# Sukikui/PTI-LDM-VAE

Hardware: AMD Instinct MI355X
Metric: vae_train_images_per_sec_256x256 (higher is better)
Workload: dtype fp16 forward operands + activations / bf16 backward operands + gradients, fp32 accumulate; 1 GPU; config/vae_dente_no_adv.json 256x256x1 batch 32/GPU: fwd + L1 + 1e-3*KL + bwd + all-reduce + Adam (perceptual term omitted: --perceptual times it; adversarial branch inactive before epoch 6, --adv times it); global_batch=32, parallelism=dp1

## Files before the change

pti_ldm_vae_amd/csrc/conv_common.h:

```cpp
#pragma once
#include "pti_common.h"

namespace pti_conv {

struct ConvArgs {
  const bf16* x;
  const unsigned char* w;
  const float* bias;
  const stat_t* in_stats;
  const float* gamma;
  const float* beta;
  const bf16* res;
  bf16* y;
  stat_t* out_stats;
  int N, H, W, Cin, Ho, Wo, Cout;
  int mode, prologue, groups, out_groups;
  float eps, inv_cnt;
  int tiles_x, tiles_y;
  int gn_mode;
  int g_groups;
  float g_inv_cnt, g_eps;
  const stat_t* g_stats; const float* g_gamma; const float* g_beta;
  float* g_sums;
  int g_T;
  bf16* act_out;
  int in_f16, res_f16, out_f16;
  int pool2;
  int relu_out;
  int w_f16;
  const bf16* x2;
  const float* p_sums;
  int x2_f16;
};
constexpr int PRO_GNB = 3;

typedef _Float16 f16x8 __attribute__((ext_vector_type(8)));
template <bool OPH>
__device__ __forceinline__ f32x16 mfma32(const bf16x8& a, const bf16x8& b, const f32x16& c) {
  if constexpr (OPH)
    return __builtin_amdgcn_mfma_f32_32x32x16_f16(__builtin_bit_cast(f16x8, a), __builtin_bit_cast(f16x8, b), c, 0, 0, 0);
  else
    return __builtin_amdgcn_mfma_f32_32x32x16_bf16(a, b, c, 0, 0, 0);
}

__host__ __device__ constexpr int pick_ck2(int cin, int ct) {
  const int ck = cin % 128 == 0 ? 128 : (cin % 64 == 0 ? 64 : 32);
  const int cap = ct >= 128 ? 128 : (ct == 64 ? 64 : 32);
  return ck < cap ? ck : cap;
}

template <int NV, int N, int O>
__device__ __forceinline__ void fold32_level(float (&v)[NV], int j) {
  if constexpr (O >= 1) {
    if constexpr (N > 1) {
      const bool hi = (j & O) != 0;
// ... 50 lines not shown
```

pti_ldm_vae_amd/csrc/conv_mfma.hip:

```cpp
#include "conv_common.h"

namespace {
using namespace pti_conv;

constexpr int TH = 8, TW = 16;

__host__ __device__ constexpr int pick_cout_tile(int cout) { return cout % 128 == 0 ? 128 : (cout % 64 == 0 ? 64 : 32); }
__host__ __device__ constexpr int pick_ck(int cin, int stride2) {
  int ck = cin % 128 == 0 ? 128 : (cin % 64 == 0 ? 64 : 32);
  return (stride2 && ck > 64) ? 64 : ck;
}
__host__ __device__ constexpr int pick_wblk(int kbc, int nt) {
  int best = 1;
  for (int w = 1; w <= kbc; ++w)
    if (kbc % w == 0 && w * nt <= 16) best = w;
  return best;
}

template <int KS, int S, int CK, int COUT_TILE>
struct Cfg {
  static constexpr int HH = (TH - 1) * S + KS, HW = (TW - 1) * S + KS;
  static constexpr int NP = HH * HW;
  static constexpr int NC = CK / 8;
  static constexpr int PIXB = CK * 2;
// ... 242 lines not shown
              b1 += __shfl_xor(b1, o, 64);
              b2 += __shfl_xor(b2, o, 64);
            }
            if (j == 0) {
              const int g = co / 2;
              stat_add(&sstat[2 * g], a1);
              stat_add(&sstat[2 * g + 1], a2);
              stat_add(&sstat[2 * g + 2], b1);
              stat_add(&sstat[2 * g + 3], b2);
            }
          }
        }
      }
    }
  }
  if (do_stats) {
    __syncthreads();
    const int g0 = (ct * COUT_TILE) / ocpg, ng = COUT_TILE / ocpg;
    if (tid < 2 * ng)
      atomicAdd((unsigned long long*)&a.out_stats[(n * a.out_groups + g0) * 2 + tid], (unsigned long long)sstat[2 * g0 + tid]);
  }
}

template <int KS, int CK, int CT, int PXF, bool SAVE, int FM, int PRO>
__global__ __launch_bounds__(256, (PXF == 2 ? 4 : 2)) void conv_mfma2_kernel(ConvArgs a) {
  using C = Cfg2<KS, CK, CT, PXF>;
  const int prologue = PRO >= 0 ? PRO : a.prologue;
  const bool gn_on = FM == 3 ? true : (FM == 0 ? a.gn_mode != 0 : false);
  const bool in_f16 = FM == 0 ? (bool)a.in_f16 : (FM == 1);
  const bool res_f16 = FM == 0 ? (bool)a.res_f16 : (FM == 1 || FM == 3);
  const bool out_f16 = FM == 0 ? (bool)a.out_f16 : (FM == 1);
  constexpr bool OPH = (FM == 1);
  if (out_f16) fp16_saturate_on();
  __shared__ __attribute__((aligned(16))) unsigned char smem[C::LDS_BYTES];
  unsigned char* halo = smem;
  const int tid = threadIdx.x, lane = tid & 63, wave = tid >> 6;
  const int hsel = lane >> 5;
  int t = blockIdx.x;
  const int tile_x = t % a.tiles_x;
  t /= a.tiles_x;
  const int tile_y = t % a.tiles_y;
  const int n = t / a.tiles_y;
  const int oy0 = tile_y * C::TH2, ox0 = tile_x * C::TW2;
  const int ct = blockIdx.y;
  const int nchunks = a.Cin / CK;
  const int wm = wave / C::WN, wn = wave % C::WN;

  const int pad_lo = (a.mode == PTI_CONV_ZINS) ? 2 : (KS - 1) / 2;
  const int vy0 = oy0 - pad_lo, vx0 = ox0 - pad_lo;
  const bool twox = (a.mode == PTI_CONV_UP2) || (a.mode == PTI_CONV_ZINS);
  const int VH = twox ? 2 * a.H : a.H, VW = twox ? 2 * a.W : a.W;

  int pbase[KS], tkey[KS];
  {
    const int j = lane & 31, tx = j & 15, row0 = 2 * PXF * wm + (j >> 4);
#pragma unroll
    for (int kw = 0; kw < KS; ++kw) {
      const int hx = tx + kw;
      tkey[kw] = (hsel ^ ((hx >> C::KEY_SHIFT) & (C::NC - 1))) << 4;
      pbase[kw] = (row0 * C::HW + hx) * C::PIXB;
    }
// ... 397 lines not shown
  }
  if (gn_on) {
    if (tid < 2 * CT) {
      const float* gsm = reinterpret_cast<const float*>(smem + C::STAT_OFF);
      float v = gsm[tid];
#pragma unroll
      for (int m = 1; m < C::WM; ++m) v += gsm[m * 2 * CT + tid];
      a.g_sums[(((size_t)n * a.g_T + tile_y * a.tiles_x + tile_x) * a.Cout + ct * CT) * 2 + tid] = v;
    }
  } else if (do_stats) {
    const stat_t* sstat = reinterpret_cast<const stat_t*>(smem + C::STAT_OFF);
    const int g0 = (ct * CT) / ocpg, ng = CT / ocpg;
    if (tid < 2 * ng)
      atomicAdd((unsigned long long*)&a.out_stats[(n * a.out_groups + g0) * 2 + tid], (unsigned long long)sstat[2 * g0 + tid]);
  }
}

template <int KS, int CK, int CT, int PXF>
int launch2_cfg(ConvArgs a, hipStream_t st) {
  using C = Cfg2<KS, CK, CT, PXF>;
  a.tiles_x = cdiv(a.Wo, C::TW2);
  a.tiles_y = cdiv(a.Ho, C::TH2);
  a.g_T = a.tiles_x * a.tiles_y;
  dim3 grid(a.N * a.tiles_x * a.tiles_y, a.Cout / CT);
  const bool res = a.res != nullptr;
  const int fm = (a.w_f16 && a.in_f16 && a.out_f16 && (a.res_f16 || !res)) ? 1
               : (!a.in_f16 && !a.out_f16 && (!a.res_f16 || !res)) ? 2
               : (!a.in_f16 && !a.out_f16 && a.res_f16) ? 3 : 0;
  const bool fwd_silu = fm == 1 && a.prologue == PTI_PRO_GN_SILU && !a.gn_mode && !a.pool2;
  const bool fwd_plain = fm == 1 && a.prologue == PTI_PRO_NONE && !a.gn_mode && !a.pool2;
  const bool dgrad = fm == 2 && a.prologue == PTI_PRO_NONE && !a.gn_mode && !a.out_stats;
  const bool dgrad_gn = fm == 3 && a.prologue == PTI_PRO_NONE && a.gn_mode && !a.out_stats && !a.pool2;
  if (a.x2) {
    if constexpr (KS == 3 && PXF == 4 && CT == 128) {
      if (!(fm == 3 && a.gn_mode && a.act_out && !a.out_stats && !a.pool2 && a.mode == PTI_CONV_S1 && !a.relu_out)) return 4;
      PTI_LAUNCH((conv_mfma2_kernel<KS, CK, CT, PXF, true, 3, PRO_GNB>), grid, dim3(256), 0, st, a);
      return 0;
    } else {
      return 4;
    }
  }
  if (a.relu_out && !(fwd_plain && !a.act_out)) return 3;
  constexpr int FPRO = PXF == 4 ? PTI_PRO_GN_SILU : -1;
  const bool fwd_gn_rt = fm == 1 && a.prologue == PTI_PRO_GN && !a.gn_mode && !a.pool2 && FPRO < 0;
  if constexpr (KS == 3) {
    if (a.act_out) {
      if (fwd_silu || fwd_gn_rt) PTI_LAUNCH((conv_mfma2_kernel<KS, CK, CT, PXF, true, 1, FPRO>), grid, dim3(256), 0, st, a);
      else if (a.w_f16) return 2;
      else PTI_LAUNCH((conv_mfma2_kernel<KS, CK, CT, PXF, true, 0, -1>), grid, dim3(256), 0, st, a);
      return 0;
    }
  } else if (a.act_out) {
    return 1;
  }
  if (fwd_silu) PTI_LAUNCH((conv_mfma2_kernel<KS, CK, CT, PXF, false, 1, FPRO>), grid, dim3(256), 0, st, a);
  else if (fwd_plain) PTI_LAUNCH((conv_mfma2_kernel<KS, CK, CT, PXF, false, 1, PTI_PRO_NONE>), grid, dim3(256), 0, st, a);
  else if (fm == 1 && !a.gn_mode && !a.pool2) PTI_LAUNCH((conv_mfma2_kernel<KS, CK, CT, PXF, false, 1, -1>), grid, dim3(256), 0, st, a);
  else if (a.w_f16) return 2;
  else if (dgrad) PTI_LAUNCH((conv_mfma2_kernel<KS, CK, CT, PXF, false, 2, PTI_PRO_NONE>), grid, dim3(256), 0, st, a);
  else if (dgrad_gn) PTI_LAUNCH((conv_mfma2_kernel<KS, CK, CT, PXF, false, 3, PTI_PRO_NONE>), grid, dim3(256), 0, st, a);
  else PTI_LAUNCH((conv_mfma2_kernel<KS, CK, CT, PXF, false, 0, -1>), grid, dim3(256), 0, st, a);
  return 0;
}
template <int KS>
int launch2(const ConvArgs& a, int ck, int ct, hipStream_t st) {
  if (ct == 128) {
    if (ck == 128) return launch2_cfg<KS, 128, 128, 4>(a, st);
    if (ck == 64) return launch2_cfg<KS, 64, 128, 4>(a, st);
    return launch2_cfg<KS, 32, 128, 4>(a, st);
  }
  if (ct == 64) {
    if (ck == 64) return launch2_cfg<KS, 64, 64, 2>(a, st);
    return launch2_cfg<KS, 32, 64, 2>(a, st);
  }
  return launch2_cfg<KS, 32, 32, 2>(a, st);
}

struct PackArgs {
  const float* src[4];
  int nsrc;
  bf16* dst;
  int cout_l, cin_l;
  int cout_o, cin_o;
  int ks, ck, cout_tile, flip;
  int f16;
  long long total;
// ... 302 lines not shown
```

pti_ldm_vae_amd/csrc/groupnorm.hip:

```cpp
#include "pti_common.h"

namespace {

__global__ __launch_bounds__(256) void gn_stats_kernel(const bf16* __restrict__ x, stat_t* __restrict__ stats,
                                                       int HW, int C, int G, int pix_per_block, int x_f16) {
  extern __shared__ stat_t sm_q[];
  stat_t* sm = sm_q;
  const int n = blockIdx.y;
  const int tid = threadIdx.x;
  const int NC = C / 8;
  const int ppi = 256 / NC;
  const int lc = tid % NC, lp = tid / NC;
  for (int i = tid; i < 2 * G; i += 256) sm[i] = 0;
  __syncthreads();
  const int p0 = blockIdx.x * pix_per_block;
  const int p1 = min(p0 + pix_per_block, HW);
  float s[8], q[8];
#pragma unroll
  for (int j = 0; j < 8; ++j) s[j] = q[j] = 0.f;
  const bf16* base = x + (size_t)n * HW * C + lc * 8;
  int p = p0 + lp;
  for (; p + 3 * ppi < p1; p += 4 * ppi) {
    u32x4 r[4];
#pragma unroll
// ... 62 lines not shown
  int bps = cdiv(2048, n);
  int ppb = cdiv(hw, bps);
  if (ppb < 16 * ppi) ppb = 16 * ppi;
  ppb = cdiv(ppb, 4 * ppi) * 4 * ppi;
  bps = cdiv(hw, ppb);
  PTI_LAUNCH(gn_stats_kernel, dim3(bps, n), dim3(256), 2 * groups * sizeof(stat_t), (hipStream_t)s,
                     (const bf16*)x, (stat_t*)stats, hw, c, groups, ppb, x_f16);
  PTI_CHECK_LAUNCH("gn_stats");
  return PTI_OK;
}

namespace {

struct GnbArgs {
  const bf16* x; const bf16* da; const bf16* dres; bf16* dx;
  const stat_t* stats; const float* gamma; const float* beta;
  float* sums;
  float* dgamma; float* dbeta;
  int HW, C, G, silu, ppb;
  float eps, inv_cnt;
  int x_f16;
  int N;
  float* part;
};

__global__ __launch_bounds__(256) void gn_bwd_reduce_kernel(GnbArgs a) {
  extern __shared__ float sm[];
  const int n = blockIdx.y, tid = threadIdx.x;
  const int NC = a.C / 8, ppi = 256 / NC, lc = tid % NC, lp = tid / NC;
  for (int i = tid; i < 8 * a.C; i += 256) sm[i] = 0.f;
  __syncthreads();
  const int cpg = a.C / a.G;
  float sc[8], sh[8], mu[8], rs[8];
#pragma unroll
  for (int j = 0; j < 8; ++j) {
    const int ch = lc * 8 + j, g = ch / cpg;
    const float sum = stat_f(a.stats, (n * a.G + g) * 2), sq = stat_f(a.stats, (n * a.G + g) * 2 + 1);
    const float mean = sum * a.inv_cnt;
    const float rstd = rsqrtf(fmaxf(sq * a.inv_cnt - mean * mean, 0.f) + a.eps);
    mu[j] = mean; rs[j] = rstd;
    sc[j] = rstd * a.gamma[ch];
    sh[j] = a.beta[ch] - mean * sc[j];
  }
  float s1[8], s2[8];
#pragma unroll
  for (int j = 0; j < 8; ++j) s1[j] = s2[j] = 0.f;
// ... 68 lines not shown
    const float* p = part + (size_t)n * T * R + i;
    int t = w;
    for (; t + 48 < T; t += 64) {
      const float a0 = p[(size_t)t * R], a1 = p[(size_t)(t + 16) * R], a2 = p[(size_t)(t + 32) * R], a3 = p[(size_t)(t + 48) * R];
      v += (a0 + a1) + (a2 + a3);
    }
    for (; t < T; t += 16) v += p[(size_t)t * R];
  }
  red[w][lane] = v;
  __syncthreads();
  if (w == 0 && i < R) {
    float r[16];
#pragma unroll
    for (int k = 0; k < 16; ++k) r[k] = red[k][lane];
#pragma unroll
    for (int o = 8; o > 0; o >>= 1)
#pragma unroll
      for (int k = 0; k < o; ++k) r[k] += r[k + o];
    sums[(size_t)n * R + i] = r[0];
  }
}

__global__ __launch_bounds__(256) void gn_bwd_apply_kernel(GnbArgs a) {
  const int n = blockIdx.y, tid = threadIdx.x;
  const int NC = a.C / 8, ppi = 256 / NC, lc = tid % NC, lp = tid / NC;
  const int cpg = a.C / a.G;
  const int p0 = blockIdx.x * a.ppb, p1 = min(p0 + a.ppb, a.HW);
  const size_t base = (size_t)n * a.HW * a.C + lc * 8;
  constexpr int U = 4;
  u32x4 rx[U], rd[U], rr[U];
  auto load_batch = [&](int pb) {
#pragma unroll
    for (int u = 0; u < U; ++u) {
      const int p = pb + u * ppi;
      rx[u] = rd[u] = rr[u] = u32x4{0u, 0u, 0u, 0u};
      if (p < p1) {
        rx[u] = __builtin_nontemporal_load((const u32x4*)(a.x + base + (size_t)p * a.C));
        rd[u] = __builtin_nontemporal_load((const u32x4*)(a.da + base + (size_t)p * a.C));
        if (a.dres) rr[u] = __builtin_nontemporal_load((const u32x4*)(a.dres + base + (size_t)p * a.C));
      }
    }
  };
  if (p0 + lp < p1) load_batch(p0 + lp);
  float sc[8], sh[8], mu[8], rs[8], ga[8], c1[8], c2[8];
#pragma unroll
  for (int j = 0; j < 8; ++j) {
    const int ch = lc * 8 + j, g = ch / cpg;
    const float sum = stat_f(a.stats, (n * a.G + g) * 2), sq = stat_f(a.stats, (n * a.G + g) * 2 + 1);
    const float mean = sum * a.inv_cnt;
    const float rstd = rsqrtf(fmaxf(sq * a.inv_cnt - mean * mean, 0.f) + a.eps);
// ... 13 lines not shown
    }
  }
  if (cpg <= 8) {
    float w1[8], w2[8];
#pragma unroll
    for (int j = 0; j < 8; ++j) {
      const f32x2 sv = *(const f32x2*)(a.sums + ((size_t)n * a.C + lc * 8 + j) * 2);
      w1[j] = ga[j] * sv[0];
      w2[j] = ga[j] * sv[1];
    }
#pragma unroll
    for (int j = 0; j < 8; ++j) {
      float t1 = 0.f, t2 = 0.f;
#pragma unroll
      for (int jj = 0; jj < 8; ++jj) {
        const bool same = (jj / cpg) == (j / cpg);
        t1 += same ? w1[jj] : 0.f;
        t2 += same ? w2[jj] : 0.f;
      }
      c1[j] = t1 * a.inv_cnt;
      c2[j] = t2 * a.inv_cnt;
    }
  }
  if (blockIdx.x == 0 && n == 0) {
    for (int i = tid; i < a.C; i += 256) {
      float d1 = 0.f, d2 = 0.f;
      for (int m = 0; m < a.N; ++m) {
        d1 += a.sums[((size_t)m * a.C + i) * 2];
        d2 += a.sums[((size_t)m * a.C + i) * 2 + 1];
      }
      if (a.dbeta) a.dbeta[i] += d1;
      if (a.dgamma) a.dgamma[i] += d2;
    }
  }
  for (int pb = p0 + lp; pb < p1; pb += U * ppi) {
    if (pb != p0 + lp) load_batch(pb);
#pragma unroll
    for (int u = 0; u < U; ++u) {
      const int p = pb + u * ppi;
      float fx[8], fd[8], fr[8], o[8];
      unpack8f(rx[u], fx, a.x_f16);
      unpack8(rd[u], fd);
      unpack8(rr[u], fr);
#pragma unroll
      for (int j = 0; j < 8; ++j) {
        float dy = fd[j];
        if (a.silu) dy *= dsilu_f(fx[j] * sc[j] + sh[j]);
// ... 42 lines not shown
  if (ppb_out) *ppb_out = ppb;
  return cdiv(hw, ppb);
}

extern "C" int pti_gn_bwd_blocks(int n, int hw, int c) {
  if (n <= 0 || hw <= 0 || c < 8 || (c & (c - 1)) || c > 512) return 0;
  return gn_bwd_grid(n, hw, c, nullptr);
}

extern "C" int pti_gn_bwd(const void* x, const void* da, const void* dres, void* dx, const int64_t* stats,
                          const float* gamma, const float* beta, float* sums, float* partials, float* dgamma,
                          float* dbeta, int n, int hw, int c, int groups, float eps, int silu, int x_f16, pti_stream_t s) {
  if (!x || !da || !dx || !stats || !gamma || !beta || !sums || !partials) PTI_FAIL(PTI_EINVAL, "gn_bwd: null pointer");
  if (c < 8 || c > 512 || (c & (c - 1)) || groups <= 0 || c % groups) PTI_FAIL(PTI_EUNSUPPORTED, "gn_bwd: c=%d groups=%d", c, groups);
  GnbArgs a;
  a.x = (const bf16*)x; a.da = (const bf16*)da; a.dres = (const bf16*)dres; a.dx = (bf16*)dx;
  a.stats = (const stat_t*)stats; a.gamma = gamma; a.beta = beta; a.sums = sums; a.dgamma = dgamma; a.dbeta = dbeta;
  a.HW = hw; a.C = c; a.G = groups; a.silu = silu; a.eps = eps; a.x_f16 = x_f16; a.N = n;
  a.inv_cnt = 1.0f / ((float)(c / groups) * (float)hw);
  int ppb;
  const int bps = gn_bwd_grid(n, hw, c, &ppb);
  a.ppb = ppb;
  a.part = partials;
  PTI_LAUNCH(gn_bwd_reduce_kernel, dim3(bps, n), dim3(256), 8 * c * sizeof(float), (hipStream_t)s, a);
  PTI_CHECK_LAUNCH("gn_bwd_reduce");
  PTI_LAUNCH(gn_sums_finalize_kernel, dim3(cdiv(2 * c, 64), n), dim3(1024), 0, (hipStream_t)s, partials, sums,
                     bps, 2 * c, (const float*)nullptr, (float*)nullptr, (float*)nullptr, 0, 0);
  PTI_CHECK_LAUNCH("gn_sums_finalize");
  PTI_LAUNCH(gn_bwd_apply_kernel, dim3(bps, n), dim3(256), 0, (hipStream_t)s, a);
  PTI_CHECK_LAUNCH("gn_bwd_apply");
  return PTI_OK;
}

extern "C" int pti_gn_bwd_apply(const void* x, const void* dy, const void* dres, void* dx, const int64_t* stats,
                                const float* gamma, const float* beta, const float* sums, float* dgamma, float* dbeta,
                                int n, int hw, int c, int groups, float eps, int x_f16, pti_stream_t s) {
  if (!x || !dy || !dx || !stats || !gamma || !beta || !sums) PTI_FAIL(PTI_EINVAL, "gn_bwd_apply: null pointer");
  if (c < 8 || c > 2048 || (c & (c - 1)) || groups <= 0 || c % groups) PTI_FAIL(PTI_EUNSUPPORTED, "gn_bwd_apply: c=%d groups=%d", c, groups);
  GnbArgs a;
  a.x = (const bf16*)x; a.da = (const bf16*)dy; a.dres = (const bf16*)dres; a.dx = (bf16*)dx;
  a.stats = (const stat_t*)stats; a.gamma = gamma; a.beta = beta; a.sums = const_cast<float*>(sums); a.dgamma = dgamma; a.dbeta = dbeta;
  a.HW = hw; a.C = c; a.G = groups; a.silu = 0; a.eps = eps; a.x_f16 = x_f16; a.N = n;
  a.inv_cnt = 1.0f / ((float)(c / groups) * (float)hw);
  const int ppi = 256 / (c / 8);
  int bps = cdiv(2048, n);
  int ppb = cdiv(hw, bps);
  if (ppb < gnb_min_iters() * ppi) ppb = gnb_min_iters() * ppi;
  ppb = cdiv(ppb, ppi) * ppi;
  bps = cdiv(hw, ppb);
  a.ppb = ppb;
  PTI_LAUNCH(gn_bwd_apply_kernel, dim3(bps, n), dim3(256), 0, (hipStream_t)s, a);
  PTI_CHECK_LAUNCH("gn_bwd_apply");
  return PTI_OK;
}

namespace {
__global__ __launch_bounds__(256) void gn_affine_grads_kernel(const float* __restrict__ sums, float* __restrict__ dgamma,
                                                              float* __restrict__ dbeta, int n, int c) {
  const int i = blockIdx.x * 256 + threadIdx.x;
  if (i >= c) return;
  float d1 = 0.f, d2 = 0.f;
  for (int m = 0; m < n; ++m) {
    const f32x2 sv = *(const f32x2*)(sums + ((size_t)m * c + i) * 2);
    d1 += sv[0];
    d2 += sv[1];
  }
  if (dbeta) dbeta[i] += d1;
  if (dgamma) dgamma[i] += d2;
}
}

extern "C" int pti_gn_affine_grads(const float* sums, float* dgamma, float* dbeta, int n, int c, pti_stream_t s) {
  if (!sums || n <= 0 || c <= 0) PTI_FAIL(PTI_EINVAL, "gn_affine_grads: bad args");
// ... 33 lines not shown
```

pti_ldm_vae_amd/csrc/pti_common.h:

```cpp
#pragma once
#include <hip/hip_runtime.h>
#include <stdint.h>
#include <stdio.h>

#include "../../include/pti_vae.h"

typedef __bf16 bf16;
typedef __bf16 bf16x8 __attribute__((ext_vector_type(8)));
typedef __bf16 bf16x4 __attribute__((ext_vector_type(4)));
typedef __bf16 bf16x2 __attribute__((ext_vector_type(2)));
typedef float f32x16 __attribute__((ext_vector_type(16)));
typedef float f32x4 __attribute__((ext_vector_type(4)));
typedef float f32x2 __attribute__((ext_vector_type(2)));
typedef uint32_t u32x4 __attribute__((ext_vector_type(4)));
typedef unsigned bu32x4 __attribute__((__vector_size__(16)));
typedef uint32_t u32x2 __attribute__((ext_vector_type(2)));
typedef short s16x4 __attribute__((ext_vector_type(4)));

void pti_set_error(const char* fmt, ...);
#define PTI_FAIL(code, ...)      \
  do {                           \
    pti_set_error(__VA_ARGS__);  \
    return (code);               \
  } while (0)
extern thread_local const void* pti_last_kernel;
#define PTI_LAUNCH(kernel, grid, block, shmem, stream, ...)                     \
// ... 177 lines not shown
  return v;
}
template <class T>
__device__ __forceinline__ T wave_max(T v) {
#pragma unroll
  for (int o = 32; o > 0; o >>= 1) v = max(v, __shfl_xor(v, o, 64));
  return v;
}

template <int WAVES, class T>
__device__ __forceinline__ T block_sum(T v, T* red) {
  const int tid = threadIdx.x;
  const T w = wave_sum(v);
  __syncthreads();
  if ((tid & 63) == 0) red[tid >> 6] = w;
  __syncthreads();
  T t = red[0];
#pragma unroll
  for (int wv = 1; wv < WAVES; ++wv) t += red[wv];
  return t;
}

static inline int cdiv(int a, int b) { return (a + b - 1) / b; }
```

pti_ldm_vae_amd/csrc/wgrad_mfma.hip:

```cpp
#include "pti_common.h"

namespace {

constexpr int TH = 8, TW = 16;
constexpr int PTI_WGRAD_SLAB_V4 = 1 << 30;
#ifndef PTI_WGRAD_BATCH_MAX
#define PTI_WGRAD_BATCH_MAX 16
#endif

struct WgArgs {
  const bf16* x;
  const bf16* dy;
  const stat_t* in_stats;
  const float* gamma;
  const float* beta;
  float* slab;
  int N, H, W, Cin, Ho, Wo, Cout;
  int mode, prologue, groups;
  float eps, inv_cnt;
  int tiles_x, tiles_y, ntiles, S;
  int ci_tiles;
  long long slab_stride;
  int x_f16;
  int diag;
};

template <int KS, int S_, int CO_T, int CI_T>
struct WCfg {
  static constexpr int HH = (TH - 1) * S_ + KS, HW = (TW - 1) * S_ + KS;
  static constexpr int NP = HH * HW;
  static constexpr int KK = KS * KS;
  static constexpr int PA = CI_T * 2 + (CI_T == 64 ? 64 : 0);
  static constexpr int PD = CO_T * 2 + (CO_T == 64 ? 64 : 0);
  static constexpr int NCA = CI_T / 8, NCD = CO_T / 8;
  static constexpr int WCO = CO_T / 32, WCI = CI_T / 32, WPX = 4 / (WCO * WCI);
  static constexpr int A_BYTES = NP * PA, D_BYTES = TH * TW * PD;
  static constexpr int HIT = (NP * NCA + 255) / 256, DIT = (TH * TW * NCD + 255) / 256;
  static constexpr int RED_BYTES = (WPX > 1) ? 32 * 32 * 4 * (WPX - 1) * WCO * WCI : 0;
  static constexpr int LDS_BYTES = (A_BYTES + D_BYTES) > RED_BYTES ? (A_BYTES + D_BYTES) : RED_BYTES;
};

template <int KS, int S_, int CO_T, int CI_T, bool PLAIN>
__global__ __launch_bounds__(256, 2) void wgrad_mfma_kernel(WgArgs a) {
  using C = WCfg<KS, S_, CO_T, CI_T>;
  const int prologue = PLAIN ? PTI_PRO_NONE : a.prologue;
  typedef short v4s __attribute__((ext_vector_type(4)));
  __shared__ __attribute__((aligned(16))) unsigned char smem[C::LDS_BYTES];
  unsigned char* lA = smem;
  unsigned char* lD = smem + C::A_BYTES;

  const int tid = threadIdx.x, lane = tid & 63, wave = tid >> 6;
  const int split = blockIdx.y;
  const int cot = blockIdx.x / a.ci_tiles, cit = blockIdx.x % a.ci_tiles;
  const int wco = wave / (C::WCI * C::WPX), wci = (wave / C::WPX) % C::WCI, wpx = wave % C::WPX;

  const int pad_lo = (a.mode == PTI_CONV_S2PAD) ? 0 : (KS - 1) / 2;
  const bool twox = (a.mode == PTI_CONV_UP2);
  const int VH = twox ? 2 * a.H : a.H, VW = twox ? 2 * a.W : a.W;

  const int g = lane >> 4, q = (lane & 15) >> 2, pp = lane & 3;
  const int pk = 8 * (g >> 1) + q;
  const int chl = 16 * (g & 1) + 4 * pp;
  const int dbase = pk * C::PD + (wco * 32 + chl) * 2;
  const int abase = (pk * S_) * C::PA + (wci * 32 + chl) * 2;

  f32x16 acc[C::KK];
#pragma unroll
  for (int t = 0; t < C::KK; ++t)
#pragma unroll
    for (int r = 0; r < 16; ++r) acc[t][r] = 0.f;

  const int alc = tid % C::NCA, alp = tid / C::NCA;
  constexpr int APSTEP = 256 / C::NCA;
  const int dlc = tid % C::NCD, dlp = tid / C::NCD;
  constexpr int DPSTEP = 256 / C::NCD;
  const int cpg = a.Cin / (a.groups > 0 ? a.groups : 1);
  float bsum[8];
#pragma unroll
  for (int j = 0; j < 8; ++j) bsum[j] = 0.f;

  u32x4 araw[C::HIT], draw[C::DIT];
  bool aok[C::HIT];
  int cur_n = -1;
  float sc[8], sh[8];

  auto issue_loads = [&](int tile) {
    int t = tile;
    const int tx_ = t % a.tiles_x; t /= a.tiles_x;
    const int ty_ = t % a.tiles_y;
    const int n = t / a.tiles_y;
    const int oy0 = ty_ * TH, ox0 = tx_ * TW;
    const int vy0 = oy0 * S_ - pad_lo, vx0 = ox0 * S_ - pad_lo;
#pragma unroll
    for (int it = 0; it < C::HIT; ++it) {
      const int p = alp + it * APSTEP;
      const int hy = p / C::HW, hx = p - hy * C::HW;
      const int vy = vy0 + hy, vx = vx0 + hx;
      const bool v = (p < C::NP) && vy >= 0 && vy < VH && vx >= 0 && vx < VW;
      const int iy = twox ? (vy >> 1) : vy, ix = twox ? (vx >> 1) : vx;
      aok[it] = v;
      araw[it] = u32x4{0u, 0u, 0u, 0u};
      if (v) araw[it] = *(const u32x4*)(a.x + ((size_t)(n * a.H + iy) * a.W + ix) * a.Cin + cit * CI_T + alc * 8);
    }
#pragma unroll
    for (int it = 0; it < C::DIT; ++it) {
      const int p = dlp + it * DPSTEP;
      const int ty = p / TW, tx = p % TW;
      const int oy = oy0 + ty, ox = ox0 + tx;
      draw[it] = u32x4{0u, 0u, 0u, 0u};
      if (p < TH * TW && oy < a.Ho && ox < a.Wo)
        draw[it] = *(const u32x4*)(a.dy + ((size_t)(n * a.Ho + oy) * a.Wo + ox) * a.Cout + cot * CO_T + dlc * 8);
    }
    return n;
  };

  auto write_lds = [&](int n) {
    if (prologue != PTI_PRO_NONE && n != cur_n) {
      cur_n = n;
#pragma unroll
      for (int j = 0; j < 8; ++j) {
        const int ch = cit * CI_T + alc * 8 + j;
        const int gg = ch / cpg;
        const float sum = stat_f(a.in_stats, (n * a.groups + gg) * 2), sq = stat_f(a.in_stats, (n * a.groups + gg) * 2 + 1);
        const float mean = sum * a.inv_cnt;
        const float rstd = rsqrtf(fmaxf(sq * a.inv_cnt - mean * mean, 0.f) + a.eps);
        sc[j] = rstd * a.gamma[ch];
        sh[j] = a.beta[ch] - mean * sc[j];
      }
    }
#pragma unroll
    for (int it = 0; it < C::HIT; ++it) {
      const int p = alp + it * APSTEP;
      if (p < C::NP) {
        u32x4 r = araw[it];
        if (prologue != PTI_PRO_NONE && aok[it]) {
          float f[8];
          unpack8f(r, f, a.x_f16);
#pragma unroll
          for (int j = 0; j < 8; ++j) {
// ... 5 lines not shown
        } else if (a.x_f16) {
          float f[8];
          unpack8f(r, f, true);
          r = pack8(f);
        }
        *(u32x4*)(lA + p * C::PA + alc * 16) = r;
      }
    }
#pragma unroll
    for (int it = 0; it < C::DIT; ++it) {
      const int p = dlp + it * DPSTEP;
      if (p < TH * TW) {
        *(u32x4*)(lD + p * C::PD + dlc * 16) = draw[it];
        if (cit == 0) {
          float f[8];
          unpack8(draw[it], f);
#pragma unroll
          for (int j = 0; j < 8; ++j) bsum[j] += f[j];
        }
      }
    }
  };

  int tile = split;
  int n_next = -1;
  if (tile < a.ntiles) n_next = issue_loads(tile);
  for (; tile < a.ntiles; tile += a.S) {
    write_lds(n_next);
    __syncthreads();
    const int nxt = tile + a.S;
    if (nxt < a.ntiles) n_next = issue_loads(nxt);
#pragma unroll
    for (int rr = 0; rr < TH / C::WPX; ++rr) {
      const int row = wpx + rr * C::WPX;
      const unsigned char* dptr = lD + dbase + row * TW * C::PD;
      const v4s d0 = __builtin_amdgcn_ds_read_tr16_b64_v4i16((v4s __attribute__((address_space(3)))*)(dptr));
      const v4s d1 = __builtin_amdgcn_ds_read_tr16_b64_v4i16((v4s __attribute__((address_space(3)))*)(dptr + 4 * C::PD));
      bf16x8 dfrag;
      {
        typedef short v8s __attribute__((ext_vector_type(8)));
        v8s t8 = {d0[0], d0[1], d0[2], d0[3], d1[0], d1[1], d1[2], d1[3]};
        dfrag = __builtin_bit_cast(bf16x8, t8);
      }
#pragma unroll
      for (int kh = 0; kh < KS; ++kh) {
#pragma unroll
        for (int kw = 0; kw < KS; ++kw) {
          const unsigned char* aptr = lA + abase + ((row * S_ + kh) * C::HW + kw) * C::PA;
          const v4s a0 = __builtin_amdgcn_ds_read_tr16_b64_v4i16((v4s __attribute__((address_space(3)))*)(aptr));
          const v4s a1 = __builtin_amdgcn_ds_read_tr16_b64_v4i16((v4s __attribute__((address_space(3)))*)(aptr + 4 * S_ * C::PA));
          typedef short v8s __attribute__((ext_vector_type(8)));
          v8s t8 = {a0[0], a0[1], a0[2], a0[3], a1[0], a1[1], a1[2], a1[3]};
          const bf16x8 afrag = __builtin_bit_cast(bf16x8, t8);
          acc[kh * KS + kw] = __builtin_amdgcn_mfma_f32_32x32x16_bf16(dfrag, afrag, acc[kh * KS + kw], 0, 0, 0);
        }
      }
    }
    __syncthreads();
  }

  float* slab = a.slab + (size_t)split * a.slab_stride;
  const int ci = cit * CI_T + wci * 32 + (lane & 31);
  const int hsel = lane >> 5;
  float* red = reinterpret_cast<float*>(smem);
#pragma unroll
  for (int t = 0; t < C::KK; ++t) {
    if constexpr (C::WPX > 1) {
      if (wpx > 0) {
        float* dst = red + (((wco * C::WCI + wci) * (C::WPX - 1) + (wpx - 1)) * 16) * 64;
#pragma unroll
        for (int r = 0; r < 16; ++r) dst[r * 64 + lane] = acc[t][r];
      }
      __syncthreads();
      if (wpx == 0) {
#pragma unroll
        for (int o = 0; o < C::WPX - 1; ++o) {
          const float* src = red + (((wco * C::WCI + wci) * (C::WPX - 1) + o) * 16) * 64;
#pragma unroll
          for (int r = 0; r < 16; ++r) acc[t][r] += src[r * 64 + lane];
        }
      }
// ... 1064 lines not shown
  if (sg == 0 && e < total + Cout) {
    f32x4 sum = red[0][col];
#pragma unroll
    for (int g = 1; g < 16; ++g) sum += red[g][col];
    if (e < total) {
      const int ci = e % Cin;
      const int co = (e / Cin) % Cout;
      const int t = e / ((long long)Cin * Cout);
#pragma unroll
      for (int j = 0; j < 4; ++j) {
        const size_t o = ((size_t)co * Cin + ci + j) * KK + t;
        dw[o] = accumulate ? dw[o] + sum[j] : sum[j];
      }
    } else if (dbias) {
      const int co = (int)(e - total);
#pragma unroll
      for (int j = 0; j < 4; ++j) dbias[co + j] = accumulate ? dbias[co + j] + sum[j] : sum[j];
    }
  }
}

template <int KS, int S_, int CO_T, int CI_T>
void launch_w(const WgArgs& a, int grid_y, hipStream_t st) {
  if (a.prologue == PTI_PRO_NONE)
    PTI_LAUNCH((wgrad_mfma_kernel<KS, S_, CO_T, CI_T, true>), dim3(grid_y, a.S), dim3(256), 0, st, a);
  else
    PTI_LAUNCH((wgrad_mfma_kernel<KS, S_, CO_T, CI_T, false>), dim3(grid_y, a.S), dim3(256), 0, st, a);
}
template <int KS, int S_>
void launch_wt(const WgArgs& a, int co_t, int ci_t, int grid_y, hipStream_t st) {
  if (co_t == 64 && ci_t == 64) launch_w<KS, S_, 64, 64>(a, grid_y, st);
  else if (co_t == 64) launch_w<KS, S_, 64, 32>(a, grid_y, st);
  else if (ci_t == 64) launch_w<KS, S_, 32, 64>(a, grid_y, st);
  else launch_w<KS, S_, 32, 32>(a, grid_y, st);
}

}

static int w6_mode(int n, int h, int w, int cin, int cout) {
  const char* e = getenv("PTI_WGRAD_V6");
  const int v = e ? atoi(e) : 3;
  if (v >= 1 && cout % 128 == 0 && cin % 64 == 0) return 2;
  if (v >= 2 && cout % 64 == 0 && cin % 64 == 0 && (v == 2 || (long long)h * w <= 128 * 128)) return 3;
  return 0;
}
static void w4_fill_job(W4Job& a, const void* x, const void* dy, int n, int h, int w, int cin, int cout, int mode) {
  a.x = (const bf16*)x; a.dy = (const bf16*)dy; a.slab = nullptr;
  a.N = n; a.H = h; a.W = w; a.Cin = cin; a.Cout = cout;
  a.tiles_x = cdiv(w, TW); a.tiles_y = cdiv(h, mode == 2 ? W6A::TH_ : TH); a.ntiles = n * a.tiles_x * a.tiles_y;
  a.slab_stride = (long long)9 * cout * cin + cout;
// ... 98 lines not shown
static int wgrad_check(const void* x, const void* dy, const int64_t* in_stats, const float* gamma, const float* beta,
                       const void* workspace, const pti_conv_desc* d) {
  if (!x || !dy || !workspace || !d) PTI_FAIL(PTI_EINVAL, "conv_wgrad_mfma: null pointer");
  if (d->cin % 32 || d->cout % 32) PTI_FAIL(PTI_EUNSUPPORTED, "conv_wgrad_mfma: cin=%d cout=%d", d->cin, d->cout);
  if (d->ksize != 1 && d->ksize != 3) PTI_FAIL(PTI_EUNSUPPORTED, "conv_wgrad_mfma: ksize");
  if (d->mode == PTI_CONV_ZINS || (d->ksize == 1 && d->mode != PTI_CONV_S1)) PTI_FAIL(PTI_EUNSUPPORTED, "conv_wgrad_mfma: mode %d", d->mode);
  if (d->prologue != PTI_PRO_NONE && (!in_stats || !gamma || !beta || d->groups <= 0 || d->cin % d->groups))
    PTI_FAIL(PTI_EINVAL, "conv_wgrad_mfma: prologue args");
  return PTI_OK;
}

extern "C" int pti_conv_wgrad_mfma_partials(const void* x, const void* dy, const int64_t* in_stats, const float* gamma,
                                            const float* beta, void* workspace, int64_t workspace_bytes,
                                            const pti_conv_desc* d, int* splits_out, pti_stream_t s) {
  if (!splits_out) PTI_FAIL(PTI_EINVAL, "conv_wgrad_mfma_partials: null splits_out");
  if (int rc = wgrad_check(x, dy, in_stats, gamma, beta, workspace, d)) return rc;
  WgArgs a;
  a.x = (const bf16*)x; a.dy = (const bf16*)dy; a.in_stats = (const stat_t*)in_stats; a.gamma = gamma; a.beta = beta;
  a.slab = (float*)workspace;
  a.N = d->n; a.H = d->h; a.W = d->w; a.Cin = d->cin; a.Ho = d->ho; a.Wo = d->wo; a.Cout = d->cout;
  a.mode = d->mode; a.prologue = d->prologue; a.groups = d->groups; a.eps = d->eps; a.x_f16 = d->in_f16;
  static const int diag_env = wgrad_diag_env();
  a.diag = diag_env;
  a.inv_cnt = d->prologue != PTI_PRO_NONE ? 1.0f / ((float)(d->cin / d->groups) * (float)d->h * (float)d->w) : 0.f;
  a.tiles_x = cdiv(d->wo, TW); a.tiles_y = cdiv(d->ho, TH); a.ntiles = d->n * a.tiles_x * a.tiles_y;
  int co_t = d->cout % 64 == 0 ? 64 : 32, ci_t = d->cin % 64 == 0 ? 64 : 32;
  if ((long long)a.ntiles * (d->cout / co_t) * (d->cin / ci_t) < 16 * 512) co_t = ci_t = 32;
  const bool v3 = d->ksize == 3 && d->mode != PTI_CONV_S2PAD;
  static const int cob_env = getenv("PTI_WGRAD_COB") ? atoi(getenv("PTI_WGRAD_COB")) : 0;
  const bool cob_ok = d->cout % 64 == 0 && d->mode == PTI_CONV_S1;
  const int cob = (cob_ok && cob_env != 1 && (cob_env == 2 || d->prologue != PTI_PRO_NONE)) ? 2 : 1;
  if (v3) { ci_t = 32; co_t = 32 * cob; }
  a.ci_tiles = d->cin / ci_t;
  const int tiles_cc = (d->cout / co_t) * a.ci_tiles;
  const int kk = d->ksize * d->ksize;
  a.slab_stride = (long long)kk * d->cout * d->cin + d->cout;
  const long long smax = workspace_bytes / (a.slab_stride * 4);
  const bool plain = d->prologue == PTI_PRO_NONE && cob == 1;
  static const int v1_wgs = getenv("PTI_WGRAD_V1_WGS") ? atoi(getenv("PTI_WGRAD_V1_WGS")) : 512;
  int S = (v3 ? (cob == 2 ? 512 : (plain ? (tiles_cc == 1 ? 1024 : 1280) : 768)) : v1_wgs) / tiles_cc;
  if (S > a.ntiles / 4) S = a.ntiles / 4;
  const int scap = v3 ? (plain ? 1024 : 512) : 256;
  if (S > scap) S = scap;
  if (S < 1) S = 1;
  if (S > smax) S = (int)smax;
  if (S < 1) PTI_FAIL(PTI_EINVAL, "conv_wgrad_mfma: workspace too small (%lld bytes per split needed)", a.slab_stride * 4);
// ... 130 lines not shown
```

Measured before the change: 2710 images/s.

## Remap workgroup order across XCDs for conv and wgrad kernels; add optional orderings

```diff
diff --git a/pti_ldm_vae_amd/csrc/conv_common.h b/pti_ldm_vae_amd/csrc/conv_common.h
--- a/pti_ldm_vae_amd/csrc/conv_common.h
+++ b/pti_ldm_vae_amd/csrc/conv_common.h
@@ -31,6 +31,7 @@
   const bf16* x2;
   const float* p_sums;
   int x2_f16;
+  int xcd_order;
 };
 constexpr int PRO_GNB = 3;
 
diff --git a/pti_ldm_vae_amd/csrc/conv_mfma.hip b/pti_ldm_vae_amd/csrc/conv_mfma.hip
--- a/pti_ldm_vae_amd/csrc/conv_mfma.hip
+++ b/pti_ldm_vae_amd/csrc/conv_mfma.hip
@@ -288,6 +288,8 @@
   }
 }
 
+__host__ __device__ constexpr bool conv2_xcd_capable(int fm, int pro) { return !(fm == 1 && pro < 0); }
+
 template <int KS, int CK, int CT, int PXF, bool SAVE, int FM, int PRO>
 __global__ __launch_bounds__(256, (PXF == 2 ? 4 : 2)) void conv_mfma2_kernel(ConvArgs a) {
   using C = Cfg2<KS, CK, CT, PXF>;
@@ -303,6 +305,12 @@
   const int tid = threadIdx.x, lane = tid & 63, wave = tid >> 6;
   const int hsel = lane >> 5;
   int t = blockIdx.x;
+  if constexpr (conv2_xcd_capable(FM, PRO)) {
+    if (a.xcd_order) {
+      t = xcd_logical(t, a.N * a.tiles_x * a.tiles_y);
+      if (t < 0) return;
+    }
+  }
   const int tile_x = t % a.tiles_x;
   t /= a.tiles_x;
   const int tile_y = t % a.tiles_y;
@@ -746,7 +754,15 @@
   a.tiles_x = cdiv(a.Wo, C::TW2);
   a.tiles_y = cdiv(a.Ho, C::TH2);
   a.g_T = a.tiles_x * a.tiles_y;
-  dim3 grid(a.N * a.tiles_x * a.tiles_y, a.Cout / CT);
+  const bool xcd_on = (pti_work_order() & PTI_WORK_ORDER_CONV) != 0;
+  const int gtiles = a.N * a.tiles_x * a.tiles_y;
+  dim3 grid(gtiles, a.Cout / CT);
+#define PTI_LAUNCH2(SAVE, FM, PRO)                                                                  \
+  do {                                                                                              \
+    a.xcd_order = xcd_on && conv2_xcd_capable(FM, PRO);                                             \
+    grid.x = a.xcd_order ? xcd_grid(gtiles) : gtiles;                                               \
+    PTI_LAUNCH((conv_mfma2_kernel<KS, CK, CT, PXF, SAVE, FM, PRO>), grid, dim3(256), 0, st, a);     \
+  } while (0)
   const bool res = a.res != nullptr;
   const int fm = (a.w_f16 && a.in_f16 && a.out_f16 && (a.res_f16 || !res)) ? 1
                : (!a.in_f16 && !a.out_f16 && (!a.res_f16 || !res)) ? 2
@@ -758,7 +774,7 @@
   if (a.x2) {
     if constexpr (KS == 3 && PXF == 4 && CT == 128) {
       if (!(fm == 3 && a.gn_mode && a.act_out && !a.out_stats && !a.pool2 && a.mode == PTI_CONV_S1 && !a.relu_out)) return 4;
-      PTI_LAUNCH((conv_mfma2_kernel<KS, CK, CT, PXF, true, 3, PRO_GNB>), grid, dim3(256), 0, st, a);
+      PTI_LAUNCH2(true, 3, PRO_GNB);
       return 0;
     } else {
       return 4;
@@ -769,23 +785,24 @@
   const bool fwd_gn_rt = fm == 1 && a.prologue == PTI_PRO_GN && !a.gn_mode && !a.pool2 && FPRO < 0;
   if constexpr (KS == 3) {
     if (a.act_out) {
-      if (fwd_silu || fwd_gn_rt) PTI_LAUNCH((conv_mfma2_kernel<KS, CK, CT, PXF, true, 1, FPRO>), grid, dim3(256), 0, st, a);
+      if (fwd_silu || fwd_gn_rt) PTI_LAUNCH2(true, 1, FPRO);
       else if (a.w_f16) return 2;
-      else PTI_LAUNCH((conv_mfma2_kernel<KS, CK, CT, PXF, true, 0, -1>), grid, dim3(256), 0, st, a);
+      else PTI_LAUNCH2(true, 0, -1);
       return 0;
     }
   } else if (a.act_out) {
     return 1;
   }
-  if (fwd_silu) PTI_LAUNCH((conv_mfma2_kernel<KS, CK, CT, PXF, false, 1, FPRO>), grid, dim3(256), 0, st, a);
-  else if (fwd_plain) PTI_LAUNCH((conv_mfma2_kernel<KS, CK, CT, PXF, false, 1, PTI_PRO_NONE>), grid, dim3(256), 0, st, a);
-  else if (fm == 1 && !a.gn_mode && !a.pool2) PTI_LAUNCH((conv_mfma2_kernel<KS, CK, CT, PXF, false, 1, -1>), grid, dim3(256), 0, st, a);
+  if (fwd_silu) PTI_LAUNCH2(false, 1, FPRO);
+  else if (fwd_plain) PTI_LAUNCH2(false, 1, PTI_PRO_NONE);
+  else if (fm == 1 && !a.gn_mode && !a.pool2) PTI_LAUNCH2(false, 1, -1);
   else if (a.w_f16) return 2;
-  else if (dgrad) PTI_LAUNCH((conv_mfma2_kernel<KS, CK, CT, PXF, false, 2, PTI_PRO_NONE>), grid, dim3(256), 0, st, a);
-  else if (dgrad_gn) PTI_LAUNCH((conv_mfma2_kernel<KS, CK, CT, PXF, false, 3, PTI_PRO_NONE>), grid, dim3(256), 0, st, a);
-  else PTI_LAUNCH((conv_mfma2_kernel<KS, CK, CT, PXF, false, 0, -1>), grid, dim3(256), 0, st, a);
+  else if (dgrad) PTI_LAUNCH2(false, 2, PTI_PRO_NONE);
+  else if (dgrad_gn) PTI_LAUNCH2(false, 3, PTI_PRO_NONE);
+  else PTI_LAUNCH2(false, 0, -1);
   return 0;
 }
+#undef PTI_LAUNCH2
 template <int KS>
 int launch2(const ConvArgs& a, int ck, int ct, hipStream_t st) {
   if (ct == 128) {
diff --git a/pti_ldm_vae_amd/csrc/groupnorm.hip b/pti_ldm_vae_amd/csrc/groupnorm.hip
--- a/pti_ldm_vae_amd/csrc/groupnorm.hip
+++ b/pti_ldm_vae_amd/csrc/groupnorm.hip
@@ -108,6 +108,7 @@
   int x_f16;
   int N;
   float* part;
+  int rev;
 };
 
 __global__ __launch_bounds__(256) void gn_bwd_reduce_kernel(GnbArgs a) {
@@ -222,10 +223,11 @@
 }
 
 __global__ __launch_bounds__(256) void gn_bwd_apply_kernel(GnbArgs a) {
-  const int n = blockIdx.y, tid = threadIdx.x;
+  const int n = a.rev ? gridDim.y - 1 - blockIdx.y : blockIdx.y, tid = threadIdx.x;
+  const int pblk = a.rev ? gridDim.x - 1 - blockIdx.x : blockIdx.x;
   const int NC = a.C / 8, ppi = 256 / NC, lc = tid % NC, lp = tid / NC;
   const int cpg = a.C / a.G;
-  const int p0 = blockIdx.x * a.ppb, p1 = min(p0 + a.ppb, a.HW);
+  const int p0 = pblk * a.ppb, p1 = min(p0 + a.ppb, a.HW);
   const size_t base = (size_t)n * a.HW * a.C + lc * 8;
   constexpr int U = 4;
   u32x4 rx[U], rd[U], rr[U];
@@ -285,7 +287,7 @@
       c2[j] = t2 * a.inv_cnt;
     }
   }
-  if (blockIdx.x == 0 && n == 0) {
+  if (pblk == 0 && n == 0) {
     for (int i = tid; i < a.C; i += 256) {
       float d1 = 0.f, d2 = 0.f;
       for (int m = 0; m < a.N; ++m) {
@@ -374,6 +376,7 @@
   const int bps = gn_bwd_grid(n, hw, c, &ppb);
   a.ppb = ppb;
   a.part = partials;
+  a.rev = (pti_work_order() & PTI_WORK_ORDER_GNB) != 0;
   PTI_LAUNCH(gn_bwd_reduce_kernel, dim3(bps, n), dim3(256), 8 * c * sizeof(float), (hipStream_t)s, a);
   PTI_CHECK_LAUNCH("gn_bwd_reduce");
   PTI_LAUNCH(gn_sums_finalize_kernel, dim3(cdiv(2 * c, 64), n), dim3(1024), 0, (hipStream_t)s, partials, sums,
@@ -401,6 +404,8 @@
   ppb = cdiv(ppb, ppi) * ppi;
   bps = cdiv(hw, ppb);
   a.ppb = ppb;
+  a.part = nullptr;
+  a.rev = (pti_work_order() & PTI_WORK_ORDER_GNB) != 0;
   PTI_LAUNCH(gn_bwd_apply_kernel, dim3(bps, n), dim3(256), 0, (hipStream_t)s, a);
   PTI_CHECK_LAUNCH("gn_bwd_apply");
   return PTI_OK;
diff --git a/pti_ldm_vae_amd/csrc/pti_common.h b/pti_ldm_vae_amd/csrc/pti_common.h
--- a/pti_ldm_vae_amd/csrc/pti_common.h
+++ b/pti_ldm_vae_amd/csrc/pti_common.h
@@ -2,6 +2,7 @@
 #include <hip/hip_runtime.h>
 #include <stdint.h>
 #include <stdio.h>
+#include <stdlib.h>
 
 #include "../../include/pti_vae.h"
 
@@ -225,3 +226,18 @@
 }
 
 static inline int cdiv(int a, int b) { return (a + b - 1) / b; }
+
+static inline int xcd_grid(int L) { return 8 * ((L + 7) / 8); }
+__device__ __forceinline__ int xcd_logical(int id, int L) {
+  const int per = (L + 7) >> 3;
+  const int i = (id & 7) * per + (id >> 3);
+  return i < L ? i : -1;
+}
+#define PTI_WORK_ORDER_WGRAD 1
+#define PTI_WORK_ORDER_CONV 2
+#define PTI_WORK_ORDER_GNB 4
+#define PTI_WORK_ORDER_DEFAULT (PTI_WORK_ORDER_WGRAD | PTI_WORK_ORDER_CONV)
+static inline int pti_work_order() {
+  const char* e = getenv("PTI_WORK_ORDER");
+  return e ? atoi(e) : PTI_WORK_ORDER_DEFAULT;
+}
diff --git a/pti_ldm_vae_amd/csrc/wgrad_mfma.hip b/pti_ldm_vae_amd/csrc/wgrad_mfma.hip
--- a/pti_ldm_vae_amd/csrc/wgrad_mfma.hip
+++ b/pti_ldm_vae_amd/csrc/wgrad_mfma.hip
@@ -6,6 +6,9 @@
 constexpr int PTI_WGRAD_SLAB_V4 = 1 << 30;
 #ifndef PTI_WGRAD_BATCH_MAX
 #define PTI_WGRAD_BATCH_MAX 16
+#endif
+#ifndef PTI_WGRAD_V1_DB
+#define PTI_WGRAD_V1_DB 0
 #endif
 
 struct WgArgs {
@@ -23,6 +26,7 @@
   long long slab_stride;
   int x_f16;
   int diag;
+  int xcd_order;
 };
 
 template <int KS, int S_, int CO_T, int CI_T>
@@ -37,7 +41,10 @@
   static constexpr int A_BYTES = NP * PA, D_BYTES = TH * TW * PD;
   static constexpr int HIT = (NP * NCA + 255) / 256, DIT = (TH * TW * NCD + 255) / 256;
   static constexpr int RED_BYTES = (WPX > 1) ? 32 * 32 * 4 * (WPX - 1) * WCO * WCI : 0;
-  static constexpr int LDS_BYTES = (A_BYTES + D_BYTES) > RED_BYTES ? (A_BYTES + D_BYTES) : RED_BYTES;
+  static constexpr bool DB = PTI_WGRAD_V1_DB && (KS == 1) && !(CO_T == 64 && CI_T == 64);
+  static constexpr int STAGE_BYTES = A_BYTES + D_BYTES;
+  static constexpr int TILE_BYTES = (DB ? 2 : 1) * STAGE_BYTES;
+  static constexpr int LDS_BYTES = TILE_BYTES > RED_BYTES ? TILE_BYTES : RED_BYTES;
 };
 
 template <int KS, int S_, int CO_T, int CI_T, bool PLAIN>
@@ -50,8 +57,15 @@
   unsigned char* lD = smem + C::A_BYTES;
 
   const int tid = threadIdx.x, lane = tid & 63, wave = tid >> 6;
-  const int split = blockIdx.y;
-  const int cot = blockIdx.x / a.ci_tiles, cit = blockIdx.x % a.ci_tiles;
+  int split = blockIdx.y, cc = blockIdx.x;
+  if (a.xcd_order) {
+    const int tiles_cc = a.ci_tiles * (a.Cout / CO_T);
+    const int logical = xcd_logical(blockIdx.x, a.S * tiles_cc);
+    if (logical < 0) return;
+    split = logical / tiles_cc;
+    cc = logical - split * tiles_cc;
+  }
+  const int cot = cc / a.ci_tiles, cit = cc % a.ci_tiles;
   const int wco = wave / (C::WCI * C::WPX), wci = (wave / C::WPX) % C::WCI, wpx = wave % C::WPX;
 
   const int pad_lo = (a.mode == PTI_CONV_S2PAD) ? 0 : (KS - 1) / 2;
@@ -79,12 +93,13 @@
 #pragma unroll
   for (int j = 0; j < 8; ++j) bsum[j] = 0.f;
 
-  u32x4 araw[C::HIT], draw[C::DIT];
-  bool aok[C::HIT];
+  constexpr int NSET = C::DB ? 2 : 1;
+  u32x4 araw_s[NSET][C::HIT], draw_s[NSET][C::DIT];
+  bool aok_s[NSET][C::HIT];
   int cur_n = -1;
   float sc[8], sh[8];
 
-  auto issue_loads = [&](int tile) {
+  auto issue_loads = [&](int tile, u32x4 (&araw)[C::HIT], u32x4 (&draw)[C::DIT], bool (&aok)[C::HIT]) {
     int t = tile;
     const int tx_ = t % a.tiles_x; t /= a.tiles_x;
     const int ty_ = t % a.tiles_y;
@@ -114,7 +129,8 @@
     return n;
   };
 
-  auto write_lds = [&](int n) {
+  auto write_lds = [&](int n, const u32x4 (&araw)[C::HIT], const u32x4 (&draw)[C::DIT], const bool (&aok)[C::HIT],
+                       unsigned char* lA, unsigned char* lD) {
     if (prologue != PTI_PRO_NONE && n != cur_n) {
       cur_n = n;
 #pragma unroll
@@ -166,14 +182,7 @@
     }
   };
 
-  int tile = split;
-  int n_next = -1;
-  if (tile < a.ntiles) n_next = issue_loads(tile);
-  for (; tile < a.ntiles; tile += a.S) {
-    write_lds(n_next);
-    __syncthreads();
-    const int nxt = tile + a.S;
-    if (nxt < a.ntiles) n_next = issue_loads(nxt);
+  auto mfma_tile = [&](const unsigned char* lA, const unsigned char* lD) {
 #pragma unroll
     for (int rr = 0; rr < TH / C::WPX; ++rr) {
       const int row = wpx + rr * C::WPX;
@@ -200,7 +209,51 @@
         }
       }
     }
+  };
+
+  int tile = split;
+  if constexpr (C::DB) {
+    int nn[2] = {-1, -1};
+    int ld = split;
+    if (ld < a.ntiles) nn[0] = issue_loads(ld, araw_s[0], draw_s[0], aok_s[0]);
+    ld += a.S;
+    if (ld < a.ntiles) nn[1] = issue_loads(ld, araw_s[1], draw_s[1], aok_s[1]);
+    ld += a.S;
+    if (tile < a.ntiles) {
+      write_lds(nn[0], araw_s[0], draw_s[0], aok_s[0], smem, smem + C::A_BYTES);
+      if (ld < a.ntiles) nn[0] = issue_loads(ld, araw_s[0], draw_s[0], aok_s[0]);
+      ld += a.S;
+    }
+    while (tile < a.ntiles) {
+#pragma unroll
+      for (int u = 0; u < 2; ++u) {
+        if (tile >= a.ntiles) break;
+        const int o = 1 - u;
+        unsigned char* stage_u = smem + u * C::STAGE_BYTES;
+        unsigned char* stage_o = smem + o * C::STAGE_BYTES;
+        __syncthreads();
+        const int nxt = tile + a.S;
+        if (nxt < a.ntiles) {
+          write_lds(nn[o], araw_s[o], draw_s[o], aok_s[o], stage_o, stage_o + C::A_BYTES);
+          if (ld < a.ntiles) nn[o] = issue_loads(ld, araw_s[o], draw_s[o], aok_s[o]);
+          ld += a.S;
+        }
+        mfma_tile(stage_u, stage_u + C::A_BYTES);
+        tile = nxt;
+      }
+    }
     __syncthreads();
+  } else {
+    int n_next = -1;
+    if (tile < a.ntiles) n_next = issue_loads(tile, araw_s[0], draw_s[0], aok_s[0]);
+    for (; tile < a.ntiles; tile += a.S) {
+      write_lds(n_next, araw_s[0], draw_s[0], aok_s[0], lA, lD);
+      __syncthreads();
+      const int nxt = tile + a.S;
+      if (nxt < a.ntiles) n_next = issue_loads(nxt, araw_s[0], draw_s[0], aok_s[0]);
+      mfma_tile(lA, lD);
+      __syncthreads();
+    }
   }
 
   float* slab = a.slab + (size_t)split * a.slab_stride;
@@ -1311,10 +1364,11 @@
 
 template <int KS, int S_, int CO_T, int CI_T>
 void launch_w(const WgArgs& a, int grid_y, hipStream_t st) {
+  const dim3 grid = a.xcd_order ? dim3(xcd_grid(grid_y * a.S)) : dim3(grid_y, a.S);
   if (a.prologue == PTI_PRO_NONE)
-    PTI_LAUNCH((wgrad_mfma_kernel<KS, S_, CO_T, CI_T, true>), dim3(grid_y, a.S), dim3(256), 0, st, a);
+    PTI_LAUNCH((wgrad_mfma_kernel<KS, S_, CO_T, CI_T, true>), grid, dim3(256), 0, st, a);
   else
-    PTI_LAUNCH((wgrad_mfma_kernel<KS, S_, CO_T, CI_T, false>), dim3(grid_y, a.S), dim3(256), 0, st, a);
+    PTI_LAUNCH((wgrad_mfma_kernel<KS, S_, CO_T, CI_T, false>), grid, dim3(256), 0, st, a);
 }
 template <int KS, int S_>
 void launch_wt(const WgArgs& a, int co_t, int ci_t, int grid_y, hipStream_t st) {
@@ -1459,6 +1513,7 @@
   a.mode = d->mode; a.prologue = d->prologue; a.groups = d->groups; a.eps = d->eps; a.x_f16 = d->in_f16;
   static const int diag_env = wgrad_diag_env();
   a.diag = diag_env;
+  a.xcd_order = (pti_work_order() & PTI_WORK_ORDER_WGRAD) != 0;
   a.inv_cnt = d->prologue != PTI_PRO_NONE ? 1.0f / ((float)(d->cin / d->groups) * (float)d->h * (float)d->w) : 0.f;
   a.tiles_x = cdiv(d->wo, TW); a.tiles_y = cdiv(d->ho, TH); a.ntiles = d->n * a.tiles_x * a.tiles_y;
   int co_t = d->cout % 64 == 0 ? 64 : 32, ci_t = d->cin % 64 == 0 ? 64 : 32;
```

Result: no change. 2734 images/s, median of 6 (+0.9%).
